# 3DAnimals/3DAnimals

Hardware: AMD Instinct MI355X
Metric: train images/sec fwd+bwd @256x256 b16 (higher is better)
Workload: dtype f32

## Files before the change

### 3danimals_amd/_lib.py

```python
from __future__ import annotations

import ctypes
import os

import torch

_HERE = os.path.dirname(os.path.abspath(__file__))
LIB_PATH = os.environ.get("A3D_LIB") or os.path.join(_HERE, "lib", "liba3d_hip.so")

_c_int, _c_float, _c_size_t, _p = ctypes.c_int, ctypes.c_float, ctypes.c_size_t, ctypes.c_void_p

SIGNATURES = {
    "a3d_version": (_c_int, []),
    "a3d_last_error": (ctypes.c_char_p, []),
    "a3d_bw_probe_fill": (_c_int, [_p, ctypes.c_int64, _p]),
    "a3d_bw_probe_read": (_c_int, [_p, ctypes.c_int64, _p, _p]),
    "a3d_dmtet_scratch_bytes": (_c_size_t, [_c_int, _c_int]),
    "a3d_dmtet_count": (_c_int, [_p, _p, _p, _c_int, _c_int, _p, _p, _p, _c_int, _c_int, _p, _p, _c_int, _p, _c_int, _p]),
    "a3d_dmtet_count_ordered": (_c_int, [_p, _c_int, _c_int, _c_int, _p, _p, _p, _p, _c_int, _p, _c_int, _p]),
    "a3d_dmtet_word_group_slots": (_c_int, []),
    "a3d_dmtet_word_group_bits": (_c_int, []),
    "a3d_dmtet_block_items": (_c_int, []),
    "a3d_dmtet_vertex_scratch_bytes": (_c_size_t, [_c_int]),
    "a3d_dmtet_gather_rows": (_c_int, [_p, _p, ctypes.c_int64, ctypes.c_int64, _c_int, _p, _p]),
    "a3d_dmtet_emit": (_c_int, [_p, _p, _p, _p, _c_int, _c_int, _p, _c_int, _c_int, _c_int, _p, _p, _p, _p, _p, _p]),
    "a3d_dmtet_emit_sparse": (_c_int, [_p, _p, _p, _p, _c_int, _c_int, _p, _c_int, _c_int, _c_int, _p, _p, _p, _p, _p, _p]),
    "a3d_dmtet_bwd": (_c_int, [_p, _p, _p, _p, _p, _c_int, _c_int, _p, _p, _c_int, _p]),
    "a3d_skin_fwd": (_c_int, [_p, _c_int, _p, _c_int, _p, _c_int, _c_int, _c_int, _c_float, _p, _p, _p, _p]),
    "a3d_skin_bwd": (_c_int, [_p, _p, _c_int, _p, _c_int, _p, _c_int, _c_int, _c_int, _c_float, _p, _p, _c_int, _p]),
    "a3d_bone_transforms_fwd": (_c_int, [_p, _c_int, _p, _p, _c_int, _c_int, _c_int, _p, _p]),
    "a3d_bone_transforms_bwd": (_c_int, [_p, _p, _c_int, _p, _p, _c_int, _c_int, _c_int, _p, _p]),
    "a3d_estimate_bones": (_c_int, [_p, _p]),
    "a3d_skin_pose_max_bones": (_c_int, []),
    "a3d_skin_pose_products_floats": (_c_size_t, [_c_int, _c_int]),
    "a3d_skin_pose_fwd": (_c_int, [_p, _c_int, _p, _c_int, _p, _p, _c_int, _c_int, _c_int, _c_int, _c_float, _p, _p, _p, _p, _p]),
    "a3d_skin_pose_bwd": (_c_int, [_p, _p, _c_int, _p, _c_int, _p, _p, _p, _p, _c_int, _c_int, _c_int, _c_int, _c_float, _p, _p, _p, _c_int, _p]),
    "a3d_normals_adjacency": (_c_int, [_p, _c_int, _c_int, _p, _p, _p, _p]),
    "a3d_normals_fwd": (_c_int, [_p, _p, _p, _p, _c_int, _c_int, _c_int, _p, _p, _c_int, _p]),
    "a3d_normals_fwd_pair": (_c_int, [_p, _c_int, _p, _c_int, _p, _p, _p, _c_int, _c_int, _p, _p, _p, _p, _c_int, _p]),
    "a3d_normals_bwd": (_c_int, [_p, _c_int, _p, _p, _p, _p, _p, _c_int, _c_int, _c_int, _p, _p, _c_int, _p, _p]),
    "a3d_shade_fwd": (_c_int, [_p, _p, _c_int, _p, _p, _c_int, ctypes.c_int64, _c_int, _p, _p, _p, _p, _c_int, _p]),
    "a3d_shade_bwd": (_c_int, [_p, _p, _p, _p, _p, _c_int, _p, _c_int, _p, _c_int, ctypes.c_int64, _c_int, _p, _p, _p, _c_int, _p]),
    "a3d_shade_bwd_rows": (_c_int, [_p, _p, _p, _p, _p, ctypes.c_int64, _p, _c_int, ctypes.c_int64, _c_int, _p, _p, _c_int, ctypes.c_int64, _p]),
    "a3d_xfm_points_fwd": (_c_int, [_p, _c_int, _p, _c_int, _c_int, _c_int, _p, _p, _p]),
    "a3d_flow_delta_fwd": (_c_int, [_p, _c_int, _c_int, _c_int, _p, _p]),
    "a3d_flow_delta_bwd": (_c_int, [_p, _c_int, _p, _c_int, _c_int, _c_int, _p, _p]),
    "a3d_xfm_points_bwd": (_c_int, [_p, _c_int, _p, _c_int, _p, _c_int, _c_int, _c_int, _p, _p, _c_int, _p, _c_int, _p, _c_int, _p, _c_int, _p]),
    "a3d_cover_scratch_bytes": (_c_size_t, [_c_int, _c_int, _c_int]),
    "a3d_cover_blocks": (_c_int, [_c_int, _c_int, _c_int]),
    "a3d_cover_groups": (_c_int, [_c_int, _c_int, _c_int]),
    "a3d_cover_group_stride": (_c_int, []),
    "a3d_cover_count": (_c_int, [_p, _c_int, _c_int, _c_int, _c_int, _p, _p]),
    "a3d_cover_emit": (_c_int, [_p, _c_int, _c_int, _c_int, _c_int, _p, _p, _p, _p]),
    "a3d_rast_scratch_bytes": (_c_size_t, [_c_int, _c_int, _c_int]),
    "a3d_rast_bins_bytes": (_c_size_t, [_c_int, _c_int, _c_int, _c_int]),
    "a3d_rast_resolve": (_c_int, [_p, _c_int, _p, _c_int, _c_int, _c_int, _c_int, _c_int, _p, _p, _p, _p]),
    "a3d_rast_resolve_gbuffer_fwd": (_c_int, [_p, _c_int, _p, _c_int, _c_int, _c_int, _c_int, _c_int, _p, _p, _p, ctypes.c_int64, _p, _p, _p, _p, _p,
                                              _c_int, _p, _p, _c_int, _p, _p, _p, _p]),
    "a3d_rast_fwd": (_c_int, [_p, _c_int, _p, _c_int, _c_int, _c_int, _c_int, _c_int, _p, _p, _c_int, _p, _p]),
    "a3d_dispatch_order_probe": (_c_int, [_c_int, _c_int, _p, _p]),
    "a3d_rast_bwd": (_c_int, [_p, _p, _p, _c_int, _p, _c_int, _c_int, _c_int, _c_int, _c_int, _p, _p]),
    "a3d_interp_fwd": (_c_int, [_p, _c_int, _c_int, _p, _p, _c_int, _c_int, _c_int, _c_int, _c_int, _p, _p]),
    "a3d_interp_bwd": (_c_int, [_p, _p, _c_int, _c_int, _p, _p, _c_int, _c_int, _c_int, _c_int, _c_int, _p, _p, _p]),
    "a3d_mesh_topology": (_c_int, [_p, _c_int, _c_int, _p, _p, _p, _p, _p, _c_int, _p]),
    "a3d_mesh_topology_finalize_max_vertices": (_c_int, []),
    "a3d_mesh_topology_finalize": (_c_int, [_p, _c_int, _c_int, _p, _p, _p, _p, _c_int, _p]),
    "a3d_gbuffer_fwd": (_c_int, [_p, _p, _p, ctypes.c_int64, _p, _p, _p, _c_int, _c_int, _c_int, _c_int, _c_int, _c_int, _p, _p, _c_int, _p, _p, _p, _p]),
    "a3d_cover_gbuffer_fwd": (_c_int, [_p, _p, _c_int, _c_int, _c_int, _c_int, _c_int, _p, ctypes.c_int64, _p, _p, _p, _p, _p, _c_int, _p, _p, _c_int,
                                       _p, _p, _p, _p]),
    "a3d_gbuffer_bwd": (_c_int, [_p, _p, _p, _p, ctypes.c_int64, _p, _p, _p, _c_int, _p, _c_int, _c_int, _c_int, _c_int, _c_int, _p, _c_int,
                                 _c_int, _p, _c_int, _p, _p, _p]),
    "a3d_gbuffer_prior_grad": (_c_int, [_p, _c_int, _c_int, _p, _p]),
    "a3d_gemm_nn_relumask": (_c_int, [_p, _p, _p, ctypes.c_int64, _c_int, _c_int, _p, _p]),
    "a3d_harmonic_embed_fwd": (_c_int, [_p, _p, _c_int, _c_int, _c_int, ctypes.c_int64, _p, _p]),
    "a3d_harmonic_embed_bwd": (_c_int, [_p, _p, _p, _c_int, _c_int, _c_int, ctypes.c_int64, _p, _p]),
    "a3d_recon_losses_scratch_bytes": (_c_size_t, [_c_int, _c_int, _c_int]),
    "a3d_recon_losses_mask_bytes": (_c_size_t, [_c_int, _c_int, _c_int]),
    "a3d_recon_losses_columns": (_c_int, []),
    "a3d_recon_losses_fwd": (_c_int, [_p, _p, _c_int, _c_int, _p, _p, _p, _p, _p, ctypes.c_int64, _p, _c_int, _c_int, _c_int, _p, _p, _p, _p]),
    "a3d_recon_losses_bwd": (_c_int, [_p, _p, _p, _c_int, _c_int, _c_int, _p, _p, _p, _p, _p, ctypes.c_int64, _p, _c_int, _c_int, _c_int, _p, _p, _p, _p]),
    "a3d_flow_loss_scratch_bytes": (_c_size_t, [_c_int, _c_int, _c_int, _c_int]),
    "a3d_flow_loss_fwd": (_c_int, [_p, _c_int, _p, _p, _c_int, _c_int, _c_int, _c_int, _p, _p, _p, _p]),
    "a3d_flow_loss_bwd": (_c_int, [_p, _p, _p, _c_int, _p, _p, _c_int, _c_int, _c_int, _c_int, _p, _p]),
    "a3d_rows_segsum": (_c_int, [_p, _p, ctypes.c_int64, _c_int, _c_int, _p, _p]),
    "a3d_rows_add_relu_fwd": (_c_int, [_p, _p, _p, ctypes.c_int64, _c_int, _c_int, _p]),
    "a3d_rows_add_relu_bwd": (_c_int, [_p, _p, _p, ctypes.c_int64, _c_int, _c_int, _p, _p, _p]),
    "a3d_aa_hash_bytes": (_c_size_t, [_c_int]),
    "a3d_aa_shards": (_c_int, []),
    "a3d_aa_capacity": (_c_int, [_c_int, _c_int, _c_int]),
    "a3d_aa_topology": (_c_int, [_p, _c_int, _c_int, _p, _p, _p]),
    "a3d_aa_topology_from_lists": (_c_int, [_p, _c_int, _p, _p, _p, _c_int, _p]),
    "a3d_aa_analyze": (_c_int, [_p, _p, _c_int, _p, _p, _c_int, _c_int, _c_int, _c_int, _c_int, _p, _p, _c_int, _p, _c_int, _p, _p, _c_int, _p]),
    "a3d_aa_fwd": (_c_int, [_p, _c_int, _p, _p, _c_int, _c_int, _c_int, _c_int, _p, _p]),
    "a3d_aa_bwd": (_c_int, [_p, _p, _c_int, _p, _p, _c_int, _p, _c_int, _p, _c_int, _c_int, _c_int, _c_int, _c_int, _p, _p, _p]),
    "a3d_composite_aa_fwd": (_c_int, [_p, _p, _p, _p, _p, _c_int, _c_int, _c_int, _c_int, _p, _p, _p]),
    "a3d_mask_aa_fwd": (_c_int, [_p, _c_int, _p, _c_int, _p, _p, _p, _c_int, _c_int, _c_int, _c_int, _p, _p]),
    "a3d_mask_aa_bwd": (_c_int, [_p, _p, _c_int, _p, _c_int, _p, _p, _c_int, _p, _c_int, _p, _c_int, _c_int, _c_int, _c_int, _c_int, _p, _c_int, _p]),
    "a3d_composite_aa_bwd": (_c_int, [_p, _p, _p, ctypes.c_int64, _p, _p, _p, _c_int, _p, _c_int, _p, _c_int, _c_int, _c_int, _c_int, _c_int, _p, _p, _p]),
}



class DmtetOrder(ctypes.Structure):

    _fields_ = [("size", ctypes.c_uint32), ("group_slots", ctypes.c_int32), ("vertex_of_rank", _p), ("edges_ranked", _p), ("edge_of_row", _p),
                ("tets_ranked", _p), ("tet_of_row", _p), ("edge_groups", _p), ("tet_groups", _p)]


class RastOpts(ctypes.Structure):

    _fields_ = [("size", ctypes.c_uint32), ("lists_stride", ctypes.c_int32), ("prev_rast", _p), ("cover_scratch", _p), ("aa_screen", _p),
                ("aa_count", _p), ("topo_off", _p), ("topo_adj", _p), ("topo_opp", _p), ("normals_v_a", _p), ("normals_v_b", _p),
                ("normals_off", _p), ("normals_adj", _p), ("normals_acc_a", _p), ("normals_a", _p), ("normals_acc_b", _p), ("normals_b", _p),
                ("normals_B_a", ctypes.c_int32), ("normals_B_b", ctypes.c_int32), ("bins", _p), ("bin_cap", ctypes.c_int32), ("bins_clean", ctypes.c_int32),
                ("defer_resolve", ctypes.c_int32), ("reserved", ctypes.c_int32)]


class AaRide(ctypes.Structure):

    _fields_ = [("size", ctypes.c_uint32), ("clip_batch", ctypes.c_int32), ("rast", _p), ("screen", _p), ("tri", _p), ("opp", _p), ("off", _p),
                ("adj", _p), ("V", ctypes.c_int32), ("F", ctypes.c_int32), ("lists_stride", ctypes.c_int32), ("reserved", ctypes.c_int32)]


class CaBuffer(ctypes.Structure):

    _fields_ = [("size", ctypes.c_uint32), ("C", ctypes.c_int32), ("vals", _p), ("bg", _p), ("out", _p), ("g_out", _p), ("g_vals", _p),
                ("bg_batch", ctypes.c_int32), ("reserved", ctypes.c_int32), ("bg_channels", ctypes.c_int32), ("g_stride", ctypes.c_int32),
                ("g_channels", ctypes.c_int32), ("out_channels", ctypes.c_int32), ("vals_rows", ctypes.c_int64)]


class CaShade(ctypes.Structure):

    _fields_ = [("size", ctypes.c_uint32), ("kd_stride", ctypes.c_int32), ("gb", _p), ("par", _p), ("kd", _p), ("clear", _p),
                ("n_clear", ctypes.c_int32), ("two_sided", ctypes.c_int32), ("params", _p), ("shaded_out", _p)]


class ShadeParams(ctypes.Structure):

    _fields_ = [("size", ctypes.c_uint32), ("rot_row_stride", ctypes.c_int32), ("rot", _p), ("view", _p), ("light", _p),
                ("rot_image_stride", ctypes.c_int64), ("view_image_stride", ctypes.c_int64), ("light_image_stride", ctypes.c_int64)]


class EstimateBonesArgs(ctypes.Structure):

    _fields_ = [("size", ctypes.c_uint32), ("N", ctypes.c_int32), ("pos", _p), ("bones", _p), ("nearest", _p), ("ok", _p), ("V", ctypes.c_int32),
                ("n_body", ctypes.c_int32), ("n_leg", ctypes.c_int32), ("body_mode_y_plus", ctypes.c_int32), ("use_y_threshold", ctypes.c_int32),
                ("y_threshold", ctypes.c_float), ("attach", ctypes.c_int32 * 4), ("blend", ctypes.c_float * 17), ("ramp", ctypes.c_float * 9), ("workspace", _p)]


class GbAux(ctypes.Structure):

    _fields_ = [("size", ctypes.c_uint32), ("reserved", ctypes.c_int32), ("tex_out", _p), ("img_out", _p), ("rows", ctypes.c_int64),
                ("pad_to", ctypes.c_int64)]


class DmtetEmitOpts(ctypes.Structure):
# ... 316 lines not shown
```

### 3danimals_amd/csrc/build.py

```python
import os
import subprocess
import sys
from concurrent.futures import ThreadPoolExecutor

HERE = os.path.dirname(os.path.abspath(__file__))
PKG = os.path.dirname(HERE)
LIB_DIR = os.path.join(PKG, "lib")
LIB = os.path.join(LIB_DIR, "liba3d_hip.so")
OBJ_DIR = os.path.join(HERE, "build")

SOURCES = {
    "common.hip": [],
    "dmtet.hip": ["-ffp-contract=off"],
    "skin.hip": [],
    "bones.hip": [],
    "normals.hip": ["-ffp-contract=off"],
    "raster.hip": ["-ffp-contract=off"],
    "cover.hip": [],
    "shade.hip": ["-ffp-contract=off"],
    "interp.hip": [],
    "gbuffer.hip": [],
    "segsum.hip": [],
    "losses.hip": [],
    "embed.hip": ["-ffp-contract=off"],
    "gemm.hip": [],
    "antialias.hip": ["-ffp-contract=off"],
    "topology.hip": [],
    "xfm.hip": ["-ffp-contract=off"],
}
COMMON = ["--offload-arch=gfx950", "-O3", "-std=c++17", "-fPIC", "-fhip-fp32-correctly-rounded-divide-sqrt", "-Wall",
          "-Wno-unused-function"]


def _hipcc():
    for c in (os.environ.get("HIPCC"), "/opt/rocm/bin/hipcc", "hipcc"):
        if c and (os.path.isabs(c) and os.path.exists(c) or not os.path.isabs(c)):
            return c
    raise RuntimeError("hipcc not found")


def _stale(target, deps):
    if not os.path.exists(target):
        return True
    t = os.path.getmtime(target)
    return any(os.path.getmtime(d) > t for d in deps)


def build(force=False, verbose=True, profile=False, exp=False):
    assert not (profile and exp)
    lib = os.path.join(LIB_DIR, "liba3d_hip_prof.so") if profile else (os.path.join(LIB_DIR, "liba3d_hip_exp.so") if exp else LIB)
    obj_dir = os.path.join(OBJ_DIR, "prof") if profile else (os.path.join(OBJ_DIR, "exp") if exp else OBJ_DIR)
    os.makedirs(LIB_DIR, exist_ok=True)
    os.makedirs(obj_dir, exist_ok=True)
    hipcc = _hipcc()
    headers = sorted(os.path.join(HERE, f) for f in os.listdir(HERE) if f.endswith(".h")) + [os.path.join(os.path.dirname(PKG), "include", "a3d.h"), os.path.abspath(__file__)]
    jobs = []
    objs = []
    for src, extra in SOURCES.items():
        s = os.path.join(HERE, src)
        o = os.path.join(obj_dir, src.replace(".hip", ".o"))
        objs.append(o)
        if force or _stale(o, [s] + headers):
            jobs.append([hipcc, "-x", "hip", "-c", s, "-o", o] + COMMON + extra + (["-DA3D_PROFILE"] if profile else []) + (["-DA3D_EXPERIMENT"] if exp else []))

    def run(cmd):
        if verbose:
            print(" ".join(cmd), flush=True)
        subprocess.check_call(cmd)

    with ThreadPoolExecutor(max_workers=min(8, max(1, len(jobs)))) as ex:
        list(ex.map(run, jobs))
    if force or jobs or _stale(lib, objs):
        run([hipcc, "--offload-arch=gfx950", "-shared", "-fPIC", "-o", lib] + objs)
    return lib


if __name__ == "__main__":
    print(build(force="--force" in sys.argv, profile="--profile" in sys.argv, exp="--exp" in sys.argv))
```

### 3danimals_amd/hostnets.py

```python
from __future__ import annotations

import torch
import torch.nn as nn
import torch.nn.functional as F


REFERENCE_FORMULATION = False


def reference_formulation(enable=True):
    global REFERENCE_FORMULATION
    REFERENCE_FORMULATION = bool(enable)
    return REFERENCE_FORMULATION


def _activation(name):
    table = {"tanh": nn.Tanh, "sigmoid": nn.Sigmoid, "relu": nn.ReLU}
    if name not in table:
        raise NotImplementedError(name)
    return table[name]()


class HarmonicEmbedding(nn.Module):

    def __init__(self, n_harmonic_functions=10, scalar=1.0):
        super().__init__()
        self.frequencies = scalar * (2.0 ** torch.arange(n_harmonic_functions))
        self._on_device = {}

    def _frequencies(self, device):
        f = self._on_device.get(device)
        if f is None:
            f = self._on_device[device] = self.frequencies.to(device)
        return f

    def forward(self, x):
        freq = self.frequencies.to(x.device) if REFERENCE_FORMULATION else self._frequencies(x.device)
        ang = (x[..., None] * freq).reshape(*x.shape[:-1], -1)
        return torch.cat((ang.sin(), ang.cos()), dim=-1)


USE_FIELD_STACK = True
SPLITK_MIN_ROWS = 65536
SPLITK_PARTS = 16


class _LinearSplitK(torch.autograd.Function):

    @staticmethod
    def forward(ctx, x, weight):
        ctx.save_for_backward(x, weight)
        return x.mm(weight.t())

    @staticmethod
    def backward(ctx, g):
        x, weight = ctx.saved_tensors
        gx = g.mm(weight) if ctx.needs_input_grad[0] else None
        gw = None
        if ctx.needs_input_grad[1]:
            gw = _split_k_weight_grad(g.contiguous(), x)
        return gx, gw


def _split_k_weight_grad(g, x):
    s, m = SPLITK_PARTS, x.shape[0]
    return torch.bmm(g.view(s, m // s, g.shape[1]).transpose(1, 2), x.view(s, m // s, x.shape[1])).sum(0)


_ZERO_BIAS = {}


def _zero_bias(x, weight):
    key = (x.device, weight.shape[0])
    b = _ZERO_BIAS.get(key)
    if b is None:
        b = _ZERO_BIAS[key] = torch.zeros(weight.shape[0], dtype=x.dtype, device=x.device)
    return b


class _LinearReLUSplitK(torch.autograd.Function):

    @staticmethod
    def forward(ctx, x, weight, bias):
        y = torch._addmm_activation(_zero_bias(x, weight) if bias is None else bias, x, weight.t(), use_gelu=False)
        ctx.save_for_backward(x, weight, y)
        return y

    @staticmethod
    def backward(ctx, g):
        x, weight, y = ctx.saved_tensors
        g = torch.ops.aten.threshold_backward(g.contiguous(), y, 0)
        gx = g.mm(weight) if ctx.needs_input_grad[0] else None
        gw = _split_k_weight_grad(g, x) if ctx.needs_input_grad[1] else None
        gb = g.sum(0) if ctx.needs_input_grad[2] else None
        return gx, gw, gb


class _FieldStack(torch.autograd.Function):

    @staticmethod
    def forward(ctx, x_emb, w_in, per_image, index, w_first, *hidden):
        from . import ops

        zero = _zero_bias(x_emb, w_in)
        ys = [torch._addmm_activation(zero, x_emb, w_in.t(), use_gelu=False)]
        if w_first is not None:
            y = ys[0].mm(w_first.t())
            ops.rows_add_relu_raw_(y, per_image, index)
            ys.append(y)
        for w in hidden:
            ys.append(torch._addmm_activation(zero, ys[-1], w.t(), use_gelu=False))
        ctx.save_for_backward(x_emb, w_in, index, w_first, *hidden, *ys)
        ctx.n_hidden, ctx.n_images = len(hidden), (per_image.shape[0] if per_image is not None else 0)
        return ys[-1]

    @staticmethod
    @torch.autograd.function.once_differentiable
    def backward(ctx, g):
        from . import ops

        saved = ctx.saved_tensors
        x_emb, w_in, index, w_first = saved[:4]
        hidden, ys = saved[4:4 + ctx.n_hidden], saved[4 + ctx.n_hidden:]
        g = torch.ops.aten.threshold_backward(g.contiguous(), ys[-1], 0)
        g_hidden = []
        for i in range(ctx.n_hidden - 1, -1, -1):
            y_prev = ys[len(ys) - ctx.n_hidden - 1 + i]
            g_hidden.append(_split_k_weight_grad(g, y_prev))
            g = ops.gemm_nn_relumask(g, hidden[i], y_prev)
        g_hidden.reverse()
        g_rows = g_first = None
        if w_first is not None:
            g_rows = ops.rows_segsum_raw(g, index, ctx.n_images)
            g_first = _split_k_weight_grad(g, ys[0])
            g = ops.gemm_nn_relumask(g, w_first, ys[0])
        g_in = _split_k_weight_grad(g, x_emb)
        g_x = g.mm(w_in) if ctx.needs_input_grad[0] else None
        return (g_x, g_in, g_rows, None, g_first, *g_hidden)


def _long_list(x, weight):
    return (x.is_cuda and x.dim() == 2 and x.shape[0] >= SPLITK_MIN_ROWS and x.shape[0] % SPLITK_PARTS == 0 and x.is_contiguous()
            and x.dtype == torch.float32 and torch.is_grad_enabled() and weight.requires_grad)


def linear(x, weight, bias=None):
    if bias is None and _long_list(x, weight):
        return _LinearSplitK.apply(x, weight)
    return F.linear(x, weight, bias)


def linear_relu(x, weight, bias=None):
    if _long_list(x, weight):
        return _LinearReLUSplitK.apply(x, weight, bias)
    if (x.is_cuda and x.dim() == 2 and x.shape[0] >= SPLITK_MIN_ROWS and x.dtype == torch.float32
            and not (torch.is_grad_enabled() and (x.requires_grad or weight.requires_grad or (bias is not None and bias.requires_grad)))):
        return torch._addmm_activation(_zero_bias(x, weight) if bias is None else bias, x, weight.t(), use_gelu=False)
    return torch.relu_(F.linear(x, weight, bias))


class MLP(nn.Module):

    def __init__(self, cin, cout, num_layers, nf=256, dropout=0, activation=None):
        super().__init__()
        assert num_layers >= 1
        dims = [cin] + [nf] * (num_layers - 1) + [cout]
        layers = []
        for i in range(num_layers):
            if i > 0:
                layers.append(nn.ReLU(inplace=True))
            layers.append(nn.Linear(dims[i], dims[i + 1], bias=False))
            if dropout and 0 < i < num_layers - 1:
                layers.append(nn.Dropout(dropout))
        if activation is not None:
            layers.append(_activation(activation))
        self.network = nn.Sequential(*layers)

    def forward(self, x, first_weight=None, per_image=None, index=None):
        if REFERENCE_FORMULATION and first_weight is None:
            return self.network(x)
        layers = list(self.network)
        i = 0
        if first_weight is not None:
            assert isinstance(layers[0], nn.Linear) and layers[0].bias is None
            x = linear(x, first_weight)
            if len(layers) > 1 and isinstance(layers[1], nn.ReLU) and x.is_cuda:
                from . import ops

                x = ops.rows_add_relu_(x, per_image, index)
                i = 2
            else:
                x = x + per_image[index]
                i = 1
        while i < len(layers):
            layer = layers[i]
            if isinstance(layer, nn.Linear) and i + 1 < len(layers) and isinstance(layers[i + 1], nn.ReLU):
                x = linear_relu(x, layer.weight, layer.bias)
                i += 2
                continue
            x = linear(x, layer.weight, layer.bias) if isinstance(layer, nn.Linear) else layer(x)
            i += 1
        return x


class CoordMLP(nn.Module):

    def __init__(self, cin, cout, num_layers, nf=256, dropout=0, activation=None, min_max=None, n_harmonic_functions=10,
                 embedder_scalar=1, embed_concat_pts=True, extra_feat_dim=0, symmetrize=False, in_layer_relu=False):
        super().__init__()
        self.extra_feat_dim = extra_feat_dim
        if n_harmonic_functions > 0:
            self.embedder = HarmonicEmbedding(n_harmonic_functions, embedder_scalar)
            dim_in = cin * 2 * n_harmonic_functions + (cin if embed_concat_pts else 0)
            self.embed_concat_pts = embed_concat_pts
        else:
            self.embedder = None
            dim_in = cin
        self.in_layer = nn.Linear(dim_in, nf)
# ... 231 lines not shown
```

### 3danimals_amd/ops.py

```python
from __future__ import annotations

import ctypes
import math
import os
from collections import OrderedDict

import torch

from . import _lib
from ._lib import call, f32c, f32h, ptr, require_device, stream


class _IdentityCache:

    def __init__(self, maxsize=8):
        self.maxsize = maxsize
        self.data = OrderedDict()

    @staticmethod
    def key(t):
        return (t.data_ptr(), tuple(t.shape), t.dtype, t._version)

    def get(self, t, make):
        k = self.key(t)
# ... 1592 lines not shown
             dt0.stride(0), ptr(valid), B, H, W, ptr(both), ptr(g_shaded), ptr(g_dino), stream())
        return g_shaded, g_dino, None, None, None, None, None, None


def reconstruction_losses(shaded_nchw, dino_nchw, image_gt, dino_gt, mask_gt, mask_dt, mask_valid, return_mask=False):
    shaded = shaded_nchw.permute(0, 2, 3, 1)
    shaded = shaded if shaded.is_contiguous() else shaded.contiguous()
    dino = None
    if dino_nchw is not None:
        dino = dino_nchw.permute(0, 2, 3, 1)
        H, W, S = dino.shape[1], dino.shape[2], dino.stride(2)
        if not (dino.dtype == torch.float32 and dino.stride(3) == 1 and S >= dino.shape[3] and dino.stride(1) == W * S and dino.stride(0) == H * W * S):
            dino = dino.contiguous()
    loss, both = _ReconLosses.apply(shaded, dino, image_gt, dino_gt, mask_gt, mask_dt[:, 0], mask_dt[:, 1], mask_valid)
    return (loss, both) if return_mask else loss


class _FlowLoss(torch.autograd.Function):
    @staticmethod
    def forward(ctx, flow, flow_gt, both, B, F):
        require_device(flow, flow_gt, both, what="flow_loss")
        N, H, W = flow.shape[:3]
        assert N == B * F and F >= 2 and flow.shape[3] == 2 and flow.stride(3) == 1 and flow.stride(1) == W * flow.stride(2) \
            and flow.stride(0) == H * flow.stride(1), "flow must be the renderer's NHWC buffer (channel slice allowed)"
        flow_gt = f32c(flow_gt)
        assert flow_gt.shape == (B, F - 1, 2, H, W) and both.numel() == N * H * W
        loss = torch.empty((B, F - 1), dtype=torch.float32, device=flow.device)
        scale = torch.empty_like(loss)
        scratch = torch.empty(_lib.lib().a3d_flow_loss_scratch_bytes(B, F, H, W), dtype=torch.uint8, device=flow.device)
        call("a3d_flow_loss_fwd", ptr(flow), flow.stride(2), ptr(flow_gt), ptr(both), B, F, H, W, ptr(scratch), ptr(loss), ptr(scale), stream())
        ctx.save_for_backward(flow, flow_gt, both, scale)
        ctx.dims = (B, F, H, W)
        return loss

    @staticmethod
    def backward(ctx, g_loss):
        flow, flow_gt, both, scale = ctx.saved_tensors
        B, F, H, W = ctx.dims
        g_flow = torch.empty((B * F, H, W, 2), dtype=torch.float32, device=flow.device)
        call("a3d_flow_loss_bwd", ptr(f32h(g_loss)), ptr(scale), ptr(flow), flow.stride(2), ptr(flow_gt), ptr(both), B, F, H, W, ptr(g_flow), stream())
        return g_flow, None, None, None, None


def flow_loss(flow_nchw, flow_gt, both, batch, num_frames):
    return _FlowLoss.apply(flow_nchw.permute(0, 2, 3, 1), flow_gt, both, int(batch), int(num_frames))


class _HarmonicEmbed(torch.autograd.Function):
    @staticmethod
    def forward(ctx, x, freq, symmetrize, ones):
        require_device(x, freq, what="harmonic_embed")
        x, freq = f32c(x), f32c(freq)
        P, n = x.shape[0], freq.shape[0]
        assert x.shape == (P, 3)
        out = torch.empty((P, 3 + 6 * n + int(ones)), dtype=torch.float32, device=x.device)
        call("a3d_harmonic_embed_fwd", ptr(x), ptr(freq), n, int(symmetrize), int(ones), P, ptr(out), stream())
        ctx.save_for_backward(x, freq)
        ctx.cfg = (int(symmetrize), int(ones))
        return out

    @staticmethod
    @torch.autograd.function.once_differentiable
    def backward(ctx, g):
        x, freq = ctx.saved_tensors
        g_x = torch.empty_like(x)
        call("a3d_harmonic_embed_bwd", ptr(f32h(g)), ptr(x), ptr(freq), freq.shape[0], ctx.cfg[0], ctx.cfg[1], x.shape[0], ptr(g_x), stream())
        return g_x, None, None, None


def harmonic_embed(x, freq, symmetrize=False, ones=False):
    return _HarmonicEmbed.apply(x, freq, symmetrize, ones)


def gemm_nn_relumask(a, b, x=None):
    require_device(a, b, what="gemm_nn_relumask")
    a, b = f32c(a), f32c(b)
    M, K = a.shape
    assert b.shape == (K, 256) and K % 32 == 0 and (x is None or (x.shape == (M, 256) and x.is_contiguous() and x.dtype == torch.float32))
    c = torch.empty((M, 256), dtype=torch.float32, device=a.device)
    call("a3d_gemm_nn_relumask", ptr(a), ptr(b), ptr(x), M, 256, K, ptr(c), stream())
    return c


def _amp_wrap_functions():
    from torch.amp import custom_bwd, custom_fwd

    for obj in list(globals().values()):
        if isinstance(obj, type) and issubclass(obj, torch.autograd.Function) and obj is not torch.autograd.Function and obj.__module__ == __name__:
            obj.forward = staticmethod(custom_fwd(obj.forward, device_type="cuda", cast_inputs=torch.float32))
            obj.backward = staticmethod(custom_bwd(obj.backward, device_type="cuda"))


_amp_wrap_functions()

if _lib.GUARD:
    _lib.set_guard(_lib.GUARD)
```

### include/a3d.h

```cpp
#ifndef A3D_H
#define A3D_H
#include <stddef.h>
#include <stdint.h>

#ifdef __cplusplus
extern "C" {
#endif

#define A3D_OK 0
#define A3D_EINVAL (-1)
#define A3D_EHIP (-2)

typedef void* a3d_stream_t;

int a3d_version(void);
const char* a3d_last_error(void);

int a3d_bw_probe_fill(float* dst, int64_t n_floats, a3d_stream_t stream);
int a3d_bw_probe_read(const float* src, int64_t n_floats, float* sink, a3d_stream_t stream);

size_t a3d_dmtet_scratch_bytes(int Ne, int Nt);
int a3d_dmtet_count(const float* sdf, const int32_t* edges, const int32_t* tets, int Ne, int Nt, void* scratch,
                    int32_t* counts , void* vertex_scratch_or_null, int vertex_scratch_is_clean, int Nv,
                    const uint32_t* edge_groups_or_null, const uint32_t* tet_groups_or_null, int group_slots ,
// ... 197 lines not shown
int a3d_cover_gbuffer_fwd(const float* rast, const int32_t* tri, int B, int V, int F, int H, int W, const void* cover_scratch, int64_t P,
                          int64_t* pix, int32_t* inv_or_null, const float* v_pos, const float* v_nrm, const float* prior, int prior_batch,
                          float* out, const float* extra_or_null, int E, float* extra_out_or_null, float* g_rows_to_clear_or_null,
                          const a3d_gb_aux* aux_or_null, a3d_stream_t stream);

int a3d_rows_segsum(const float* g, const int64_t* img, int64_t P, int C, int B, float* out, a3d_stream_t stream);
int a3d_rows_add_relu_fwd(float* y , const float* rows , const int64_t* img , int64_t P, int C, int B,
                          a3d_stream_t stream);
int a3d_rows_add_relu_bwd(const float* g, const float* y, const int64_t* img, int64_t P, int C, int B, float* g_pre ,
                          float* g_rows , a3d_stream_t stream);

size_t a3d_aa_hash_bytes(int F);
int a3d_aa_shards(void);
int a3d_aa_capacity(int B, int H, int W);
int a3d_aa_topology(const int32_t* tri, int F, int V, void* hash, int32_t* opp, a3d_stream_t stream);
int a3d_aa_topology_from_lists(const int32_t* tri, int F, const int32_t* off, const int32_t* adj, int32_t* opp, int lists_stride,
                               a3d_stream_t stream);
int a3d_aa_analyze(const float* rast, const float* clip, int clip_batch, const int32_t* tri, const int32_t* opp_or_null, int B, int V,
                   int F, int H, int W, float* screen, void* work, int capacity, int32_t* count, int prepared,
                   const int32_t* off_or_null, const int32_t* adj_or_null, int lists_stride, a3d_stream_t stream);
int a3d_aa_fwd(const float* color, int C, const void* work, const int32_t* count, int capacity, int B, int H, int W, float* out,
               a3d_stream_t stream);
int a3d_aa_bwd(const float* g_out, const float* color, int C, const void* work, const int32_t* count, int capacity,
               const float* clip, int clip_batch, const int32_t* tri, int B, int V, int F, int H, int W, float* g_color,
               float* g_clip, a3d_stream_t stream);
typedef struct a3d_aa_ride {
    uint32_t size;
    int32_t clip_batch;
    const float* rast;
    const float* screen;
    const int32_t* tri;
    const int32_t* opp;
    const int32_t* off;
    const int32_t* adj;
    int32_t V;
    int32_t F;
    int32_t lists_stride;
    int32_t reserved;
} a3d_aa_ride;
typedef struct a3d_ca_shade {
    uint32_t size;
    int32_t kd_stride;
    const float* gb;
    const float* par;
    const float* kd;
    float* clear;
    int32_t n_clear;
    int32_t two_sided;
    const a3d_shade_params* params;
    float* shaded_out;
} a3d_ca_shade;
typedef struct a3d_ca_buffer {
    uint32_t size;
    int32_t C;
    const float* vals;
    const float* bg;
    float* out;
    const float* g_out;
    float* g_vals;
    int32_t bg_batch;
    int32_t reserved;
    int32_t bg_channels;
    int32_t g_stride;
    int32_t g_channels;
    int32_t out_channels;
    int64_t vals_rows;
} a3d_ca_buffer;
int a3d_composite_aa_fwd(const a3d_ca_buffer* first, const a3d_ca_buffer* second_or_null, const int32_t* inv, void* work, int32_t* count,
                         int capacity, int B, int H, int W, const a3d_aa_ride* analyze_or_null, const a3d_ca_shade* shade_or_null,
                         a3d_stream_t stream);
int a3d_mask_aa_fwd(const float* rast, int C, const float* bg_or_null, int bg_batch, float* out, void* work, int32_t* count, int capacity,
                    int B, int H, int W, const a3d_aa_ride* analyze_or_null , a3d_stream_t stream);
int a3d_mask_aa_bwd(const float* g_out, const float* rast, int C, const float* bg_or_null, int bg_batch, const void* work,
                    const int32_t* count, int capacity, const float* clip, int clip_batch, const int32_t* tri, int B, int V, int F, int H,
                    int W, float* g_clip,
                    int g_channels_first ,
                    a3d_stream_t stream);
int a3d_composite_aa_bwd(const a3d_ca_buffer* first, const a3d_ca_buffer* second_or_null, const int64_t* pix, int64_t P, const int32_t* inv,
                         const void* work, const int32_t* count, int capacity, const float* clip, int clip_batch, const int32_t* tri, int B,
                         int V, int F, int H, int W, float* g_clip, const a3d_ca_shade* shade_or_null, a3d_stream_t stream);

int a3d_gemm_nn_relumask(const float* A, const float* B, const float* X, int64_t M, int N, int K, float* C, a3d_stream_t stream);

int a3d_harmonic_embed_fwd(const float* x , const float* freq , int n, int symmetrize, int ones, int64_t P, float* out,
                           a3d_stream_t stream);
int a3d_harmonic_embed_bwd(const float* g_out, const float* x, const float* freq, int n, int symmetrize, int ones, int64_t P, float* g_x,
                           a3d_stream_t stream);

size_t a3d_recon_losses_scratch_bytes(int B, int H, int W);
size_t a3d_recon_losses_mask_bytes(int B, int H, int W);
int a3d_recon_losses_columns(void);
int a3d_recon_losses_fwd(const float* shaded, const float* dino, int D, int dino_stride, const float* image_gt, const float* dino_gt, const float* mask_gt,
                         const float* dt0, const float* dt1_or_null, int64_t dt_stride, const float* valid, int B, int H, int W, void* scratch,
                         uint8_t* both, float* loss, a3d_stream_t stream);
int a3d_recon_losses_bwd(const float* g_loss, const float* shaded, const float* dino, int D, int dino_stride, int g_dino_stride, const float* image_gt, const float* dino_gt,
                         const float* mask_gt, const float* dt0, const float* dt1_or_null, int64_t dt_stride, const float* valid, int B, int H,
                         int W, const uint8_t* both, float* g_shaded, float* g_dino, a3d_stream_t stream);
size_t a3d_flow_loss_scratch_bytes(int B, int F, int H, int W);
int a3d_flow_loss_fwd(const float* flow, int pix_stride, const float* flow_gt, const uint8_t* both, int B, int F, int H, int W, void* scratch,
                      float* loss, float* scale, a3d_stream_t stream);
int a3d_flow_loss_bwd(const float* g_loss, const float* scale, const float* flow, int pix_stride, const float* flow_gt, const uint8_t* both,
                      int B, int F, int H, int W, float* g_flow, a3d_stream_t stream);

int a3d_xfm_points_fwd(const float* points, int points_batch, const float* matrix, int matrix_batch, int B, int V, float* out,
                       float* g_matrix_to_clear_or_null, a3d_stream_t stream);
int a3d_xfm_points_bwd(const float* g_out, int g_stride, const float* points, int points_batch, const float* matrix, int matrix_batch, int B, int V,
                       float* g_points_or_null, float* g_matrix_or_null, int g_matrix_is_clear,
                       const float* g_points_addend_or_null ,
                       int addend_stride,
                       const float* g_points_addend2_or_null ,
                       int addend2_stride,
                       const float* g_out2_or_null ,
                       int g2_stride, a3d_stream_t stream);
int a3d_flow_delta_fwd(const float* clip, int N, int F, int V, float* delta, a3d_stream_t stream);
int a3d_flow_delta_bwd(const float* g_delta, int g_stride , const float* clip, int N,
                       int F, int V, float* g_clip, a3d_stream_t stream);

#ifdef __cplusplus
}
#endif
#endif
```

Measured before the change: 1022.

## Add bf16x3-split MFMA GEMM kernels for field MLP backward

After: 1089 (median of 6 runs). +6.6%, better.

```diff
diff --git a/3danimals_amd/_lib.py b/3danimals_amd/_lib.py
--- a/3danimals_amd/_lib.py
+++ b/3danimals_amd/_lib.py
@@ -72,6 +72,10 @@
                                  _c_int, _p, _c_int, _p, _p, _p]),
     "a3d_gbuffer_prior_grad": (_c_int, [_p, _c_int, _c_int, _p, _p]),
     "a3d_gemm_nn_relumask": (_c_int, [_p, _p, _p, ctypes.c_int64, _c_int, _c_int, _p, _p]),
+    "a3d_gemm_x6_nt_relu": (_c_int, [_p, _p, _p, _p, ctypes.c_int64, _p, _p]),
+    "a3d_gemm_x6_nn_relumask": (_c_int, [_p, _p, _p, ctypes.c_int64, _p, _p]),
+    "a3d_gemm_x6_tn_work_bytes": (_c_size_t, []),
+    "a3d_gemm_x6_tn": (_c_int, [_p, _p, ctypes.c_int64, _p, _p, _p]),
     "a3d_harmonic_embed_fwd": (_c_int, [_p, _p, _c_int, _c_int, _c_int, ctypes.c_int64, _p, _p]),
     "a3d_harmonic_embed_bwd": (_c_int, [_p, _p, _p, _c_int, _c_int, _c_int, ctypes.c_int64, _p, _p]),
     "a3d_recon_losses_scratch_bytes": (_c_size_t, [_c_int, _c_int, _c_int]),
diff --git a/3danimals_amd/csrc/build.py b/3danimals_amd/csrc/build.py
--- a/3danimals_amd/csrc/build.py
+++ b/3danimals_amd/csrc/build.py
@@ -24,6 +24,7 @@
     "losses.hip": [],
     "embed.hip": ["-ffp-contract=off"],
     "gemm.hip": [],
+    "gemm_x6.hip": ["-ffp-contract=off"],
     "antialias.hip": ["-ffp-contract=off"],
     "topology.hip": [],
     "xfm.hip": ["-ffp-contract=off"],
diff --git a/3danimals_amd/csrc/gemm_x6.hip b/3danimals_amd/csrc/gemm_x6.hip
--- /dev/null
+++ b/3danimals_amd/csrc/gemm_x6.hip
@@ -0,0 +1,262 @@
+#include "a3d_common.h"
+
+namespace {
+
+typedef float f32x16 __attribute__((ext_vector_type(16)));
+typedef float f32x4 __attribute__((ext_vector_type(4)));
+typedef float f32x2 __attribute__((ext_vector_type(2)));
+typedef __bf16 bf16x2 __attribute__((ext_vector_type(2)));
+typedef __bf16 bf16x8 __attribute__((ext_vector_type(8)));
+typedef unsigned u32x4 __attribute__((ext_vector_type(4)));
+
+constexpr int X6_D = 256;
+constexpr int X6_KS = 16;
+constexpr int X6_STEPS = X6_D / X6_KS;
+constexpr int X6_BM = 128;
+constexpr int X6_PLANE = 8 * 2 * 32;
+constexpr int X6_TN_SLABS = 256;
+
+__device__ __forceinline__ unsigned pk_bf16(float a, float b) {
+    const f32x2 v = {a, b};
+    return __builtin_bit_cast(unsigned, __builtin_convertvector(v, bf16x2));
+}
+__device__ __forceinline__ float bf_lo(unsigned w) { return __builtin_bit_cast(float, w << 16); }
+__device__ __forceinline__ float bf_hi(unsigned w) { return __builtin_bit_cast(float, w & 0xffff0000u); }
+
+__device__ __forceinline__ void split8(const float (&v)[8], u32x4& hp, u32x4& mp, u32x4& lp) {
+#pragma unroll
+    for (int i = 0; i < 4; ++i) {
+        const float a0 = v[2 * i], a1 = v[2 * i + 1];
+        const unsigned h = pk_bf16(a0, a1);
+        const float r0 = a0 - bf_lo(h), r1 = a1 - bf_hi(h);
+        const unsigned m = pk_bf16(r0, r1);
+        const float s0 = r0 - bf_lo(m), s1 = r1 - bf_hi(m);
+        hp[i] = h;
+        mp[i] = m;
+        lp[i] = pk_bf16(s0, s1);
+    }
+}
+
+__device__ __forceinline__ bf16x8 frag(u32x4 v) { return __builtin_bit_cast(bf16x8, v); }
+
+__device__ __forceinline__ f32x16 mfma_x6(u32x4 ah, u32x4 am, u32x4 al, u32x4 bh, u32x4 bm, u32x4 bl, f32x16 acc) {
+    acc = __builtin_amdgcn_mfma_f32_32x32x16_bf16(frag(al), frag(bh), acc, 0, 0, 0);
+    acc = __builtin_amdgcn_mfma_f32_32x32x16_bf16(frag(ah), frag(bl), acc, 0, 0, 0);
+    acc = __builtin_amdgcn_mfma_f32_32x32x16_bf16(frag(am), frag(bm), acc, 0, 0, 0);
+    acc = __builtin_amdgcn_mfma_f32_32x32x16_bf16(frag(am), frag(bh), acc, 0, 0, 0);
+    acc = __builtin_amdgcn_mfma_f32_32x32x16_bf16(frag(ah), frag(bm), acc, 0, 0, 0);
+    acc = __builtin_amdgcn_mfma_f32_32x32x16_bf16(frag(ah), frag(bh), acc, 0, 0, 0);
+    return acc;
+}
+
+__device__ __forceinline__ void stage8(u32x4* buf, int c, int i, const float (&v)[8]) {
+    u32x4 hp, mp, lp;
+    split8(v, hp, mp, lp);
+    const int f = ((c >> 5) * 2 + i) * 32 + (c & 31);
+    buf[f] = hp;
+    buf[X6_PLANE + f] = mp;
+    buf[2 * X6_PLANE + f] = lp;
+}
+
+__device__ __forceinline__ void step_x6(const u32x4* buf, int lane, u32x4 ah, u32x4 am, u32x4 al, f32x16 (&acc)[8]) {
+    const int h = lane >> 5, r = lane & 31;
+#pragma unroll
+    for (int j = 0; j < 8; ++j) {
+        const int f = (j * 2 + h) * 32 + r;
+        acc[j] = mfma_x6(ah, am, al, buf[f], buf[X6_PLANE + f], buf[2 * X6_PLANE + f], acc[j]);
+    }
+}
+
+template <int MODE>
+__global__ __launch_bounds__(256, 2) void gm_x6_rows_kernel(const float* __restrict__ A, const float* __restrict__ W, const float* __restrict__ Xm,
+                                                         const float* __restrict__ rows, const long long* __restrict__ idx, int M,
+                                                         float* __restrict__ C) {
+    __shared__ u32x4 Bs[2][3 * X6_PLANE];
+    const int tid = threadIdx.x, lane = tid & 63, wave = tid >> 6, r = lane & 31, h = lane >> 5;
+    const long long m0 = (long long)blockIdx.x * X6_BM + 32 * wave;
+    const long long arow = m0 + r < M ? m0 + r : M - 1;
+    const float* a_lane = A + arow * X6_D + 8 * h;
+    const int c = tid;
+    float wv[2][8];
+    auto load_w = [&](int s) {
+#pragma unroll
+        for (int i = 0; i < 2; ++i) {
+            const int k0 = X6_KS * s + 8 * i;
+            if (MODE == 0) {
+                const f32x4 p = *reinterpret_cast<const f32x4*>(W + c * X6_D + k0);
+                const f32x4 q = *reinterpret_cast<const f32x4*>(W + c * X6_D + k0 + 4);
+#pragma unroll
+                for (int j = 0; j < 4; ++j) {
+                    wv[i][j] = p[j];
+                    wv[i][4 + j] = q[j];
+                }
+            } else {
+#pragma unroll
+                for (int j = 0; j < 8; ++j) wv[i][j] = W[(k0 + j) * X6_D + c];
+            }
+        }
+    };
+    auto store_w = [&](u32x4* buf) {
+#pragma unroll
+        for (int i = 0; i < 2; ++i) stage8(buf, c, i, wv[i]);
+    };
+
+    f32x16 acc[8];
+#pragma unroll
+    for (int j = 0; j < 8; ++j)
+#pragma unroll
+        for (int q = 0; q < 16; ++q) acc[j][q] = 0.f;
+
+    f32x4 an0 = *reinterpret_cast<const f32x4*>(a_lane), an1 = *reinterpret_cast<const f32x4*>(a_lane + 4);
+    load_w(0);
+    store_w(Bs[0]);
+    load_w(1);
+    __syncthreads();
+#pragma unroll 1
+    for (int s = 0; s < X6_STEPS; ++s) {
+        const float av[8] = {an0[0], an0[1], an0[2], an0[3], an1[0], an1[1], an1[2], an1[3]};
+        if (s + 1 < X6_STEPS) {
+            an0 = *reinterpret_cast<const f32x4*>(a_lane + X6_KS * (s + 1));
+            an1 = *reinterpret_cast<const f32x4*>(a_lane + X6_KS * (s + 1) + 4);
+        }
+        u32x4 ah, am, al;
+        split8(av, ah, am, al);
+        step_x6(Bs[s & 1], lane, ah, am, al, acc);
+        if (s + 1 < X6_STEPS) {
+            store_w(Bs[(s + 1) & 1]);
+            if (s + 2 < X6_STEPS) load_w(s + 2);
+        }
+        __syncthreads();
+    }
+#pragma unroll
+    for (int q = 0; q < 16; ++q) {
+        const long long m = m0 + (q & 3) + 8 * (q >> 2) + 4 * h;
+        if (m < M) {
+            const float* add = (MODE == 0 && rows) ? rows + idx[m] * X6_D : nullptr;
+#pragma unroll
+            for (int j = 0; j < 8; ++j) {
+                const int n = 32 * j + r;
+                float v = acc[j][q];
+                if (MODE == 0) {
+                    if (add) v = v + add[n];
+                    v = v > 0.f ? v : 0.f;
+                } else {
+                    v = Xm[m * X6_D + n] > 0.f ? v : 0.f;
+                }
+                C[m * X6_D + n] = v;
+            }
+        }
+    }
+}
+
+__global__ __launch_bounds__(512, 1) void gm_x6_tn_kernel(const float* __restrict__ G, const float* __restrict__ Y, int M, int slab_rows,
+                                                       float* __restrict__ part) {
+    __shared__ u32x4 Bs[2][3 * X6_PLANE];
+    const int tid = threadIdx.x, lane = tid & 63, wave = tid >> 6, r = lane & 31, h = lane >> 5;
+    const long long mb = (long long)blockIdx.x * slab_rows;
+    const long long me = mb + slab_rows < M ? mb + slab_rows : M;
+    const int n_steps = me > mb ? (int)((me - mb + X6_KS - 1) / X6_KS) : 0;
+    const float* g_lane = G + 32 * wave + r;
+    const int c = tid & 255, ci = tid >> 8;
+    const float* y_thr = Y + c;
+    float gv[8], yv[8];
+    auto load = [&](int s) {
+        const long long ga = mb + X6_KS * s + 8 * h, ya = mb + X6_KS * s + 8 * ci;
+#pragma unroll
+        for (int j = 0; j < 8; ++j) {
+            gv[j] = ga + j < me ? g_lane[(ga + j) * X6_D] : 0.f;
+            yv[j] = ya + j < me ? y_thr[(ya + j) * X6_D] : 0.f;
+        }
+    };
+
+    f32x16 acc[8];
+#pragma unroll
+    for (int j = 0; j < 8; ++j)
+#pragma unroll
+        for (int q = 0; q < 16; ++q) acc[j][q] = 0.f;
+
+    if (n_steps > 0) {
+        load(0);
+        stage8(Bs[0], c, ci, yv);
+        float ga_cur[8];
+#pragma unroll
+        for (int j = 0; j < 8; ++j) ga_cur[j] = gv[j];
+        if (n_steps > 1) load(1);
+        __syncthreads();
+#pragma unroll 1
+        for (int s = 0; s < n_steps; ++s) {
+            u32x4 ah, am, al;
+            split8(ga_cur, ah, am, al);
+            step_x6(Bs[s & 1], lane, ah, am, al, acc);
+            if (s + 1 < n_steps) {
+                stage8(Bs[(s + 1) & 1], c, ci, yv);
+#pragma unroll
+                for (int j = 0; j < 8; ++j) ga_cur[j] = gv[j];
+                if (s + 2 < n_steps) load(s + 2);
+            }
+            __syncthreads();
+        }
+    }
+    float* out = part + (long long)blockIdx.x * X6_D * X6_D;
+#pragma unroll
+    for (int q = 0; q < 16; ++q) {
+        const int n = 32 * wave + (q & 3) + 8 * (q >> 2) + 4 * h;
+#pragma unroll
+        for (int j = 0; j < 8; ++j) out[n * X6_D + 32 * j + r] = acc[j][q];
+    }
+}
+
+constexpr int X6_RED_WAVES = 4, X6_RED_PER = X6_TN_SLABS / X6_RED_WAVES, X6_OUT4 = X6_D * X6_D / 4;
+__global__ __launch_bounds__(64 * X6_RED_WAVES) void gm_x6_tn_reduce_kernel(const f32x4* __restrict__ part, f32x4* __restrict__ dW) {
+    __shared__ f32x4 wsum[X6_RED_WAVES - 1][64];
+    const int lane = threadIdx.x & 63, q = threadIdx.x >> 6;
+    const int i = blockIdx.x * 64 + lane;
+    const f32x4* p = part + (long long)(q * X6_RED_PER) * X6_OUT4 + i;
+    f32x4 s = p[0];
+#pragma unroll 8
+    for (int k = 1; k < X6_RED_PER; ++k) s += p[(long long)k * X6_OUT4];
+    if (q) wsum[q - 1][lane] = s;
+    __syncthreads();
+    if (q == 0) {
+#pragma unroll
+        for (int w = 0; w < X6_RED_WAVES - 1; ++w) s += wsum[w][lane];
+        dW[i] = s;
+    }
+}
+
+}
+
+extern "C" int a3d_gemm_x6_nt_relu(const float* X, const float* W, const float* rows, const int64_t* idx, int64_t M, float* Y,
+                                   a3d_stream_t stream) {
+    A3D_CHECK_ARG(M >= 0 && M < 0x7fffffffll && (rows == nullptr) == (idx == nullptr));
+    if (M == 0) return A3D_OK;
+    A3D_CHECK_ARG(X && W && Y);
+    hipLaunchKernelGGL(gm_x6_rows_kernel<0>, dim3(a3d_div_up(M, X6_BM)), dim3(256), 0, (hipStream_t)stream, X, W, (const float*)nullptr, rows,
+                       (const long long*)idx, (int)M, Y);
+    A3D_LAUNCH_CHECK();
+    return A3D_OK;
+}
+
+extern "C" int a3d_gemm_x6_nn_relumask(const float* G, const float* W, const float* X, int64_t M, float* C, a3d_stream_t stream) {
+    A3D_CHECK_ARG(M >= 0 && M < 0x7fffffffll);
+    if (M == 0) return A3D_OK;
+    A3D_CHECK_ARG(G && W && X && C);
+    hipLaunchKernelGGL(gm_x6_rows_kernel<1>, dim3(a3d_div_up(M, X6_BM)), dim3(256), 0, (hipStream_t)stream, G, W, X, (const float*)nullptr,
+                       (const long long*)nullptr, (int)M, C);
+    A3D_LAUNCH_CHECK();
+    return A3D_OK;
+}
+
+extern "C" size_t a3d_gemm_x6_tn_work_bytes(void) { return (size_t)X6_TN_SLABS * X6_D * X6_D * sizeof(float); }
+
+extern "C" int a3d_gemm_x6_tn(const float* G, const float* Y, int64_t M, float* work, float* dW, a3d_stream_t stream) {
+    A3D_CHECK_ARG(M >= 0 && M < 0x7fffffffll);
+    A3D_CHECK_ARG(G && Y && work && dW);
+    hipStream_t s = (hipStream_t)stream;
+    const int slab_rows = (int)a3d_div_up(a3d_div_up(M, X6_TN_SLABS), X6_KS) * X6_KS;
+    hipLaunchKernelGGL(gm_x6_tn_kernel, dim3(X6_TN_SLABS), dim3(512), 0, s, G, Y, (int)M, slab_rows, work);
+    A3D_LAUNCH_CHECK();
+    hipLaunchKernelGGL(gm_x6_tn_reduce_kernel, dim3(X6_OUT4 / 64), dim3(64 * X6_RED_WAVES), 0, s, (const f32x4*)work, (f32x4*)dW);
+    A3D_LAUNCH_CHECK();
+    return A3D_OK;
+}
diff --git a/3danimals_amd/hostnets.py b/3danimals_amd/hostnets.py
--- a/3danimals_amd/hostnets.py
+++ b/3danimals_amd/hostnets.py
@@ -41,6 +41,8 @@
 
 
 USE_FIELD_STACK = True
+FIELD_GEMM = "x6"
+X6_FORWARD = False
 SPLITK_MIN_ROWS = 65536
 SPLITK_PARTS = 16
 
@@ -102,16 +104,21 @@
     def forward(ctx, x_emb, w_in, per_image, index, w_first, *hidden):
         from . import ops
 
+        assert FIELD_GEMM in ("x6", "fp32"), FIELD_GEMM
+        x6 = FIELD_GEMM == "x6" and X6_FORWARD
         zero = _zero_bias(x_emb, w_in)
         ys = [torch._addmm_activation(zero, x_emb, w_in.t(), use_gelu=False)]
         if w_first is not None:
-            y = ys[0].mm(w_first.t())
-            ops.rows_add_relu_raw_(y, per_image, index)
-            ys.append(y)
+            if x6:
+                ys.append(ops.gemm_x6_nt_relu(ys[0], w_first, per_image.contiguous(), index.contiguous()))
+            else:
+                y = ys[0].mm(w_first.t())
+                ops.rows_add_relu_raw_(y, per_image, index)
+                ys.append(y)
         for w in hidden:
-            ys.append(torch._addmm_activation(zero, ys[-1], w.t(), use_gelu=False))
+            ys.append(ops.gemm_x6_nt_relu(ys[-1], w) if x6 else torch._addmm_activation(zero, ys[-1], w.t(), use_gelu=False))
         ctx.save_for_backward(x_emb, w_in, index, w_first, *hidden, *ys)
-        ctx.n_hidden, ctx.n_images = len(hidden), (per_image.shape[0] if per_image is not None else 0)
+        ctx.n_hidden, ctx.n_images, ctx.x6 = len(hidden), (per_image.shape[0] if per_image is not None else 0), FIELD_GEMM == "x6"
         return ys[-1]
 
     @staticmethod
@@ -123,17 +130,19 @@
         x_emb, w_in, index, w_first = saved[:4]
         hidden, ys = saved[4:4 + ctx.n_hidden], saved[4 + ctx.n_hidden:]
         g = torch.ops.aten.threshold_backward(g.contiguous(), ys[-1], 0)
+        weight_grad = ops.gemm_x6_tn if ctx.x6 else _split_k_weight_grad
+        input_grad = ops.gemm_x6_nn_relumask if ctx.x6 else ops.gemm_nn_relumask
         g_hidden = []
         for i in range(ctx.n_hidden - 1, -1, -1):
             y_prev = ys[len(ys) - ctx.n_hidden - 1 + i]
-            g_hidden.append(_split_k_weight_grad(g, y_prev))
-            g = ops.gemm_nn_relumask(g, hidden[i], y_prev)
+            g_hidden.append(weight_grad(g, y_prev))
+            g = input_grad(g, hidden[i], y_prev)
         g_hidden.reverse()
         g_rows = g_first = None
         if w_first is not None:
             g_rows = ops.rows_segsum_raw(g, index, ctx.n_images)
-            g_first = _split_k_weight_grad(g, ys[0])
-            g = ops.gemm_nn_relumask(g, w_first, ys[0])
+            g_first = weight_grad(g, ys[0])
+            g = input_grad(g, w_first, ys[0])
         g_in = _split_k_weight_grad(g, x_emb)
         g_x = g.mm(w_in) if ctx.needs_input_grad[0] else None
         return (g_x, g_in, g_rows, None, g_first, *g_hidden)
diff --git a/3danimals_amd/ops.py b/3danimals_amd/ops.py
--- a/3danimals_amd/ops.py
+++ b/3danimals_amd/ops.py
@@ -1698,6 +1698,44 @@
     return c
 
 
+def _x6_operand(t, rows=None):
+    assert t.is_contiguous() and t.dtype == torch.float32 and t.dim() == 2 and t.shape[1] == 256 and (rows is None or t.shape[0] == rows), \
+        "gemm_x6: fp32 contiguous [M,256] operands"
+    return t
+
+
+def gemm_x6_nt_relu(x, w, rows=None, idx=None):
+    require_device(x, w, what="gemm_x6_nt_relu")
+    M = _x6_operand(x).shape[0]
+    _x6_operand(w, 256)
+    if rows is not None:
+        _x6_operand(rows)
+        assert idx is not None and idx.dtype == torch.int64 and idx.is_contiguous() and idx.shape == (M,)
+    y = torch.empty((M, 256), dtype=torch.float32, device=x.device)
+    call("a3d_gemm_x6_nt_relu", ptr(x), ptr(w), ptr(rows), ptr(idx), M, ptr(y), stream())
+    return y
+
+
+def gemm_x6_nn_relumask(g, w, x):
+    require_device(g, w, x, what="gemm_x6_nn_relumask")
+    M = _x6_operand(g).shape[0]
+    _x6_operand(w, 256)
+    _x6_operand(x, M)
+    c = torch.empty((M, 256), dtype=torch.float32, device=g.device)
+    call("a3d_gemm_x6_nn_relumask", ptr(g), ptr(w), ptr(x), M, ptr(c), stream())
+    return c
+
+
+def gemm_x6_tn(g, y):
+    require_device(g, y, what="gemm_x6_tn")
+    M = _x6_operand(g).shape[0]
+    _x6_operand(y, M)
+    work = torch.empty(_lib.lib().a3d_gemm_x6_tn_work_bytes() // 4, dtype=torch.float32, device=g.device)
+    dw = torch.empty((256, 256), dtype=torch.float32, device=g.device)
+    call("a3d_gemm_x6_tn", ptr(g), ptr(y), M, ptr(work), ptr(dw), stream())
+    return dw
+
+
 def _amp_wrap_functions():
     from torch.amp import custom_bwd, custom_fwd
 
diff --git a/include/a3d.h b/include/a3d.h
--- a/include/a3d.h
+++ b/include/a3d.h
@@ -303,6 +303,11 @@
 
 int a3d_gemm_nn_relumask(const float* A, const float* B, const float* X, int64_t M, int N, int K, float* C, a3d_stream_t stream);
 
+int a3d_gemm_x6_nt_relu(const float* X, const float* W, const float* rows, const int64_t* idx, int64_t M, float* Y, a3d_stream_t stream);
+int a3d_gemm_x6_nn_relumask(const float* G, const float* W, const float* X, int64_t M, float* C, a3d_stream_t stream);
+size_t a3d_gemm_x6_tn_work_bytes(void);
+int a3d_gemm_x6_tn(const float* G, const float* Y, int64_t M, float* work, float* dW, a3d_stream_t stream);
+
 int a3d_harmonic_embed_fwd(const float* x , const float* freq , int n, int symmetrize, int ones, int64_t P, float* out,
                            a3d_stream_t stream);
 int a3d_harmonic_embed_bwd(const float* g_out, const float* x, const float* freq, int n, int symmetrize, int ones, int64_t P, float* g_x,
```
